# rdevooght/sequence-based-recommendations

Hardware: AMD Instinct MI355X
Metric: user-sequences/sec training (ML-1M shape, seq200 b256) at 1/2/4/8 GPUs (higher is better)
Workload: dtype f32; 1 GPU; c2: train.py -m RNN --r_t GRU --r_l 128 --max_length 200 -b 256 --loss CCE --u_m adam, N=3706 items, Zipf(1.0) ids, lengths=full, 256 rows per GPU; global_batch=256, seq_len=200, parallelism=dp1

## Files before the change

### sequence-based-recommendations_amd/csrc/sbr_api.hip

```cpp
#include "sbr_common.h"
#include <stdarg.h>
#include <stdio.h>
#include <string.h>
#include <algorithm>
#include <stdlib.h>
#include <math.h>
#include <array>
#include <atomic>
#include <chrono>

static thread_local std::string g_err;
void sbr_set_error(const char* fmt, ...) {
    char buf[1024];
    va_list ap; va_start(ap, fmt); vsnprintf(buf, sizeof(buf), fmt, ap); va_end(ap);
    g_err = buf;
}
extern "C" const char* sbr_last_error(void) { return g_err.c_str(); }
extern "C" int sbr_abi_version(void) { return SBR_ABI_VERSION; }


int sbr_build_layout(const sbr_config& cfg, Layout& lay, std::string& err) {
    char buf[256];
#define LFAIL(...) do { snprintf(buf, sizeof(buf), __VA_ARGS__); err = buf; return SBR_EINVAL; } while (0)
    if (cfg.abi_version != SBR_ABI_VERSION) LFAIL("abi_version %d != %d", cfg.abi_version, SBR_ABI_VERSION);
// ... 338 lines not shown
    h->sw = sbr_read_switches();
    const SbrSwitches& sw = h->sw;
    h->rpt = sw.rpt;
    if (h->rpt != 1 && h->rpt != 2 && h->rpt != 4 && h->rpt != 8 && h->rpt != 16) { h->rpt = 4; while (h->rpt < 16 && h->lay.Bp / h->rpt > 256) h->rpt <<= 1; }
    if (sw.tail_trace) {
        if (hipMalloc(&h->tail_trace, 16384 * sizeof(unsigned long long)) != hipSuccess) h->tail_trace = nullptr;
        else (void)hipMemset(h->tail_trace, 0, 16384 * sizeof(unsigned long long));
    }
    int prio_lo = 0, prio_hi = 0;
    (void)hipDeviceGetStreamPriorityRange(&prio_lo, &prio_hi);
    bool ok = true;
    for (hipStream_t* st : handle_streams(h)) ok = ok && hipStreamCreateWithPriority(st, hipStreamNonBlocking, prio_hi) == hipSuccess;
    for (hipEvent_t* ev : handle_events(h)) ok = ok && hipEventCreateWithFlags(ev, hipEventDisableTiming) == hipSuccess;
#if SBR_BB_STREAM
    ok = ok && hipStreamCreateWithPriority(&h->s_bb, hipStreamNonBlocking, SBR_BB_STREAM == 2 ? prio_lo : prio_hi) == hipSuccess;
#endif
    if (!ok || hipHostMalloc((void**)&h->lag_host, 8 * sizeof(float), hipHostMallocDefault) != hipSuccess) {
        sbr_set_error("side stream creation failed"); sbr_destroy(h); return SBR_EHIP;
    }
#if !SBR_BB_STREAM
    h->s_bb = h->side3;
#endif
    memset(h->lag_host, 0, 8 * sizeof(float));
    hipError_t e = hipMemsetAsync(h->arena, 0, h->lay.s_end * sizeof(float), h->stream);
    if (e == hipSuccess) e = hipStreamSynchronize(h->stream);
    if (e != hipSuccess) { sbr_set_error("arena initialisation failed: %s", hipGetErrorString(e)); sbr_destroy(h); return SBR_EHIP; }
    if (h->lay.n_at > 0) {
        std::vector<float> at(h->lay.n_at);
        const double lr = cfg->learning_rate, b1 = cfg->beta1, b2 = cfg->beta2;
        for (int t = 1; t <= h->lay.n_at; ++t) at[t - 1] = (float)(lr * sqrt(1.0 - pow(b2, (double)t)) / (1.0 - pow(b1, (double)t)));
        e = hipMemcpy(h->A(h->lay.a_at), at.data(), at.size() * sizeof(float), hipMemcpyHostToDevice);
        if (e != hipSuccess) { sbr_set_error("a_t table upload failed: %s", hipGetErrorString(e)); sbr_destroy(h); return SBR_EHIP; }
    }
    *out = h;
    return SBR_OK;
}

extern "C" void sbr_destroy(sbr_handle* h) {
    if (!h) return;
    (void)hipStreamSynchronize(h->stream);
    for (hipStream_t* st : handle_streams(h)) if (*st) (void)hipStreamSynchronize(*st);
    for (int r = 0; r < sbr_handle::kRing; ++r)
        for (int i = 0; i < SBR_N_PHASES; ++i) if (h->ev[r][i]) (void)hipEventDestroy(h->ev[r][i]);
    for (int r = 0; r < sbr_handle::kChain; ++r)
        for (int i = 0; i < 2; ++i) if (h->ev_ch[r][i]) (void)hipEventDestroy(h->ev_ch[r][i]);
    for (hipEvent_t* ev : handle_events(h)) if (*ev) (void)hipEventDestroy(*ev);
#if SBR_BB_STREAM
    if (h->s_bb) (void)hipStreamDestroy(h->s_bb);
#endif
    for (hipStream_t* st : handle_streams(h)) if (*st) (void)hipStreamDestroy(*st);
    if (h->lag_host) (void)hipHostFree(h->lag_host);
    if (h->own_arena && h->arena) (void)hipFree(h->arena);
    if (h->tail_trace) (void)hipFree(h->tail_trace);
    if (h->tail_slab_dev) (void)hipFree(h->tail_slab_dev);
    if (h->rank_scratch) (void)hipFree(h->rank_scratch);
    delete h;
}

extern "C" int sbr_num_params(const sbr_handle* h) { return h ? (int)h->descs.size() : SBR_EINVAL; }

extern "C" int sbr_param_shape(const sbr_handle* h, int i, int64_t dims[2], int* ndim) {
    CHECK_ARG(h && dims && ndim && i >= 0 && i < (int)h->descs.size(), "bad parameter index %d", i);
    const ParamDesc& d = h->descs[i];
    dims[0] = d.d0; dims[1] = d.ndim == 2 ? d.d1 : 1; *ndim = d.ndim;
    return SBR_OK;
}

static SbrSparseRows sparse_rows(sbr_handle* h, int b) {
    const SparseBlockLayout& sb = h->lay.sparse[b];
    SbrSparseRows r; memset(&r, 0, sizeof(r));
    r.npairs = sb.npairs; r.n_rows = sb.n_rows;
    for (int k = 0; k < sb.npairs; ++k) { r.off[k] = sb.off[k]; r.width[k] = sb.width[k]; r.stride[k] = sb.stride[k]; }
    r.p = h->P(0); r.g = h->Gd(0); r.s0 = h->St(0, 0); r.s1 = h->lay.n_state_arrays > 1 ? h->St(1, 0) : nullptr;
    r.last = (int*)h->A(sb.a_last);
    return r;
}
static SbrSparseUpd sparse_upd(sbr_handle* h) {
// ... 190 lines not shown
    const double geom = sbr_tail_geom(h->sw.tail_scatter_lds);
    SbrTChunks& tc = h->tail_bounds;
    tc.n = nc;
    tc.lo[0] = 0;
    double pw = h->sw.tail_scatter_lds ? (double)kTailFirst : 1.0;
    for (int c = 0; c < nc; ++c) {
        const int rem = y.T - tc.lo[c], left = nc - c;
        const int share = (rem + left - 1) / left;
        const int n_small = nc >= 4 ? nc / 2 : (nc - 1) / 2;
        int sz = (geom > 1.0 && c < n_small) ? std::min(share, std::max(1, (int)(pw + 0.5))) : (geom > 1.0 ? share : std::min(rem, ch));
        if (c == nc - 1) sz = rem;
        sz = std::max(1, std::min(sz, rem - (left - 1)));
        tc.lo[c + 1] = tc.lo[c] + sz;
        pw *= geom > 1.0 ? geom : 1.0;
    }
    for (int c = nc; c <= SBR_TCHUNKS_MAX; ++c) tc.lo[c] = y.T;
    return nc;
}

static int tail_next_epoch(sbr_handle* h) {
    h->prog_epoch = (h->prog_epoch + 1) & 0x7FFFF; if (!h->prog_epoch) h->prog_epoch = 1;
    return h->prog_epoch;
}
static int* tail_words(sbr_handle* h, int* nwaves) {
    *nwaves = (h->lay.Bp / rec_args(h, 0).rpt) * 8;
    return (int*)h->A(h->lay.a_prog);
}

static int tail_cost_scan(sbr_handle* h) {
    const Layout& y = h->lay;
    h->tail_cost_scanned = false;
    if (!h->sw.tail_scatter_lds) return SBR_OK;
    hipError_t e = hipSuccess;
    if (launch_scatter_cost_scan(h->side2, (const int*)h->A(y.a_soff), (int*)h->A(y.a_sP), y.cfg.input_size, h->tail_nc, y.T * y.Bp * y.F,
                                 y.G * y.layer[0].Hp, kTailScatterUnits, &e)) {
        if (e != hipSuccess) { sbr_set_error("HIP launch failed: %s", hipGetErrorString(e)); return SBR_EHIP; }
        h->tail_cost_scanned = true;
    }
    return SBR_OK;
}

static inline void chain_mark(sbr_handle* h, hipStream_t st, int dir, int which) {
    if (!h->chain_timing || h->ch_n >= sbr_handle::kChain) return;
    hipEvent_t& e = h->ev_ch[h->ch_n][which];
    if (!e && hipEventCreate(&e) != hipSuccess) { e = nullptr; return; }
    (void)hipEventRecord(e, st);
// ... 155 lines not shown
                SBR_LAUNCH(launch_sparse_catch_up_batch(s, sparse_rows(h, b), sparse_upd(h), h->bX, h->blen, y.T, y.Bp, y.F, (int)h->step_count));
    h->tail_nc = h->step_open ? tail_plan(h, &h->tail_ch) : 0;
    const bool training = h->step_open;
    h->step_open = false;
    h->tail_sorted = false;
    h->set_use[h->bb_set] = ++h->batch_seq; h->bb_unread = false;
    if (training) { if (h->train_fwd_open) h->bb_slow = 2; h->train_fwd_open = true; }
    h->cells_early = false;
    bool forked = false;
    if (training && h->sw.sparse_out_early && sparse_lazy(h) && y.S > 0 && y.cfg.loss != SBR_LOSS_CCE && !SBR_LOSS_IS_MARGIN(y.cfg.loss)) {
        int kb = -1;
        for (int b = 0; b < y.n_sparse; ++b) if (y.sparse[b].kind == 1) kb = b;
        if (kb >= 0) {
            SBR_HIP(hipEventRecord(h->ev_fork, s)); forked = true;
            SBR_HIP(hipStreamWaitEvent(h->side, h->ev_fork, 0));
            int* cells = (int*)h->A(y.a_cells);
            SBR_LAUNCH(launch_build_cells(h->side, h->btgt, h->bsmp, y.Bg, y.S, cells));
            SBR_LAUNCH(launch_sparse_catch_up_list(h->side, sparse_rows(h, kb), sparse_upd(h), cells, nullptr, y.C, y.C, (int)h->step_count));
            SBR_HIP(hipEventRecord(h->ev_cells, h->side));
            h->cells_early = true;
            h->side_pending = true;
        }
    }
    if (h->tail_nc >= 2 && h->sw.tail_overlap == 1) {
        if (!forked) SBR_HIP(hipEventRecord(h->ev_fork, s));
        SBR_HIP(hipStreamWaitEvent(h->side2, h->ev_fork, 0));
        SBR_LAUNCH(launch_scatter_sort(h->side2, h->bX, h->blen, y.T, y.Bp, y.F, y.cfg.input_size, (int*)h->A(y.a_scnt),
                                       (int*)h->A(y.a_soff), (int*)h->A(y.a_scur), (int*)h->A(y.a_sid), (int*)h->A(y.a_spos), 0,
                                       h->tail_ch, h->tail_nc, &h->tail_bounds, &h->scnt_zero_n));
        h->tail_sorted = true;
        { const int rc = tail_cost_scan(h); if (rc != SBR_OK) return rc; }
    }
    if (y.D == 2) return forward_bi(h);
    for (int l = 0; l < y.L; ++l) {
        const LayerLayout& ly = y.layer[l];
        const int GHp = y.G * ly.Hp;
        RecArgs ra = rec_args(h, l);
        if (l == 0 && y.E) {
            SBR_LAUNCH(launch_gather_concat(s, h->P(y.p_Emb), h->bX, h->A(y.a_emb), y.T, y.Bp, y.F, y.Ep));
            SBR_LAUNCH(launch_gemm(s, h->A(y.a_emb), ly.n_in_p, 1, h->P(ly.p_Win), GHp, 1, h->A(ly.a_xt), GHp, y.T * y.Bp, GHp,
                                   ly.n_in_p, h->P(ly.p_b), nullptr, 0, simple_gemm(h)));
            mark(h, 1);
        } else if (l == 0) {
            if (y.F == 1 && h->sw.fuse_gather && sbr_rec_fwd_can_fuse_gather(ra, simple_rec(h))) {
                ra.gX = h->bX; ra.gWin = h->P(ly.p_Win); ra.gbias = h->P(ly.p_b);
            } else {
                SBR_LAUNCH(launch_gather_xt(s, h->P(ly.p_Win), h->P(ly.p_b), h->bX, h->A(ly.a_xt), y.T, y.Bp,
                                            y.F, GHp, h->n_rows));
            }
            mark(h, 1);
        } else {
            const LayerLayout& lo = y.layer[l - 1];
            layer_gemm_hint(h, false, false);
            SBR_LAUNCH(launch_gemm(s, h->A(lo.a_hs) + (size_t)y.Bp * lo.Hp, lo.Hp, 1, h->P(ly.p_Win), GHp, 1, h->A(ly.a_xt), GHp,
                                   y.T * y.Bp, GHp, lo.Hp, h->P(ly.p_b), nullptr, 0, simple_gemm(h)));
        }
        if (l == 0 && h->tail_sorted) ra.fence_kb = kTailFenceKb;
        SBR_LAUNCH_CHAIN(0, s, launch_rec_forward(s, ra, simple_rec(h)));
    }
    mark(h, 2);
    h->fwd_done = true;
    return SBR_OK;
}

static float* h_last(sbr_handle* h) {
    const Layout& y = h->lay; const LayerLayout& ly = y.layer[(y.L - 1) * y.D];
    if (y.D == 2) return h->A(y.a_hcat);
    return h->A(ly.a_hs) + (size_t)y.T * y.Bp * ly.Hp;
}

static int side_join(sbr_handle* h) {
    if (h->tail_join_pending) {
        SBR_HIP(hipStreamWaitEvent(h->stream, h->ev_tail2, 0));
        SBR_HIP(hipStreamWaitEvent(h->stream, h->ev_tail, 0));
        h->tail_join_pending = false; h->side_pending = false;
    }
    if (h->side_pending) {
        SBR_HIP(hipEventRecord(h->ev_join, h->side));
        SBR_HIP(hipStreamWaitEvent(h->stream, h->ev_join, 0));
        h->side_pending = false;
    }
    return SBR_OK;
}

extern "C" int sbr_loss_backward_output(sbr_handle* h) {
    CHECK_ARG(h, "null handle");
    sbr_gemm_set_exact_f32((h->lay.cfg.flags & SBR_FLAG_F32_MFMA) != 0);
    if (!h->fwd_done) { sbr_set_error("sbr_loss_backward_output: call sbr_forward first"); return SBR_ESTATE; }
    const Layout& y = h->lay; hipStream_t s = h->stream, sd = h->side;
    const int R = h->n_rows, Hp = y.HLt, N = y.N;
    const bool sg = simple_gemm(h);
    h->grads_clean = false;
    h->dh_slabs_n = 0;
    float* hl = h_last(h);
    float* ws = h->A(y.a_ws);
    float* ws2 = h->A(y.a_ws2);
    const int* tgt = h->btgt;
    if (R < y.Bp) SBR_HIP(hipMemsetAsync(h->A(y.a_dhlast), 0, (size_t)y.Bp * Hp * sizeof(float), s));
    h->side_pending = true;
    h->fill_done = false;
    h->tail_gated = false; h->last_tail_gated = 0;
    bool fill_needed = false;
    if (!simple_rec(h))
        for (int l = 0; l < y.L * y.D; ++l) fill_needed = fill_needed || sbr_rec_cluster_ok(rec_args(h, l));
    auto side_batch_work = [&]() -> int {
        if (fill_needed) {
            for (int l = 0; l < y.L * y.D; ++l) {
                RecArgs a = rec_args(h, l);
                if (sbr_rec_cluster_ok(a)) SBR_LAUNCH(sbr_rec_bwd_cl_fill(sd, a));
            }
            SBR_HIP(hipEventRecord(h->ev_fill, sd)); h->fill_done = true;
        }
        if (h->tail_nc >= 2) {
            if (h->ev_lg_rec) SBR_HIP(hipStreamWaitEvent(h->side2, h->ev_lg_rec, 0));
            if (!h->tail_sorted) {
                SBR_LAUNCH(launch_scatter_sort(h->side2, h->bX, h->blen, y.T, y.Bp, y.F, y.cfg.input_size, (int*)h->A(y.a_scnt),
                                               (int*)h->A(y.a_soff), (int*)h->A(y.a_scur), (int*)h->A(y.a_sid), (int*)h->A(y.a_spos), 0,
                                               h->tail_ch, h->tail_nc, &h->tail_bounds, &h->scnt_zero_n));
                { const int rc = tail_cost_scan(h); if (rc != SBR_OK) return rc; }
            }
        } else if (!(y.cfg.flags & SBR_FLAG_ATOMIC_SCATTER) || y.E || y.n_sparse) {
            SBR_LAUNCH(launch_scatter_sort(sd, h->bX, h->blen, y.T, y.Bp, y.F,
                                           y.cfg.input_size, (int*)h->A(y.a_scnt), (int*)h->A(y.a_soff), (int*)h->A(y.a_scur),
                                           (int*)h->A(y.a_sid), (int*)h->A(y.a_spos), y.E ? 1 : 0, 0, 1, nullptr, &h->scnt_zero_n));
            if (y.D == 2 && !y.E)
                SBR_LAUNCH(launch_scatter_sort(sd, (const int*)h->A(y.a_Xr), h->blen, y.T, y.Bp, y.F, y.cfg.input_size,
                                               (int*)h->A(y.a_s2cnt), (int*)h->A(y.a_s2off), (int*)h->A(y.a_s2cur),
                                               (int*)h->A(y.a_s2sid), (int*)h->A(y.a_s2pos), 0));
            SBR_HIP(hipEventRecord(h->ev_sort, sd));
        }
        return SBR_OK;
    };
    if (fill_needed) {
        SBR_HIP(hipEventRecord(h->ev_fork, s));
        SBR_HIP(hipStreamWaitEvent(sd, h->ev_fork, 0));
        const int rc = side_batch_work(); if (rc != SBR_OK) return rc;
    }
    auto release_side = [&]() -> int {
        const bool mark3 = h->timing && ((h->timing_marks >> 3) & 1) && h->ev[h->ring_cur][3];
        if (kTailGateFirst && h->in_train_step && h->tail_nc >= 2 && h->sw.tail_overlap == 1 && h->tail_sorted && y.L == 1 && y.D == 1 && !fill_needed && !mark3) {
            int nwaves = 0;
            int* words = tail_words(h, &nwaves);
            SBR_LAUNCH(launch_tail_gate_wave(sd, words, nwaves, tail_next_epoch(h), y.T, (int*)h->A(y.a_fault)));
            h->tail_gated = true;
            h->ev_lg_rec = nullptr; h->ev_step_rec = h->ev_fork; h->lg_seq = h->batch_seq;
        } else {
            h->ev_lg_rec = h->ev_step_rec = record_shared(h, h->ev_lg, 3); h->lg_seq = h->batch_seq;
            SBR_HIP(hipStreamWaitEvent(sd, h->ev_lg_rec, 0));
        }
        return SBR_OK;
    };
    if (y.cfg.loss == SBR_LOSS_CCE || SBR_LOSS_IS_MARGIN(y.cfg.loss)) {
        float* lg = h->A(y.a_logits);
        const int Nl = (N + 3) & ~3;
        const bool bf16p = (y.cfg.flags & SBR_FLAG_BF16_PROJECTION) && !sg;
        int keep = 0;
        bool fold = false;
        if (!sg && y.D == 1 && R == y.Bp && !simple_rec(h)) {
            RecArgs ra = rec_args(h, y.L - 1);
            fold = sbr_rec_x6p_ok(ra) && !sbr_rec_cluster_ok(ra);
        }
        bool head_done = false;
        if (h->sw.head_fuse && y.cfg.loss == SBR_LOSS_CCE && !sg && !bf16p && !(y.cfg.flags & SBR_FLAG_F32_MFMA) && y.D == 1 && R == y.Bp) {
            int nsl = 0; hipError_t he = hipSuccess;
            h->head_epoch += 1; if (!h->head_epoch) h->head_epoch = 1;
            if (launch_head_cce(s, hl, h->P(y.p_WoutT), h->P(y.p_bout), tgt, h->bpop, lg, h->A(y.a_rowcost), ws, y.ws_floats,
                                (unsigned*)h->A(y.a_hstat), (int*)h->A(y.a_fault), y.Bp, N, Nl, Hp, y.Bg, h->head_epoch, h->sw.head_wait_ticks, &nsl, &he,
                                (y.cfg.flags & SBR_FLAG_PROFILE_REC) && (size_t)y.Bp * 16 >= 256 * 8 ? (unsigned long long*)h->A(y.a_prof) + (size_t)2 * (y.Bp / 16) * 16 * 8 : nullptr)) {
                SBR_LAUNCH(he);
                head_done = true;
// ... 186 lines not shown
            if (!gated) SBR_LAUNCH(launch_tail_gate(sd, words, nwaves, a.prog_epoch, y.T, a.fault));
            {
                hipError_t we = hipSuccess;
                if (!launch_gemm_slabs_x6_poll(sd, h->A(ly.a_hs), 1, ly.Hp, a.dxt, GHp, 1, ly.Hp, GHp, K, ws2, n_slabs, GHp, slab,
                                               gru ? a.dhi : nullptr, ly.Hp, gru ? 2 * ly.Hp : 0, &we, wg_f16 ? 2 : 3, 1.0f, wg_f16 ? 512.0f : 1.0f, pl)) {
                    sbr_set_error("overlapped tail: the weight-gradient GEMM rejected the shape"); return SBR_EINVAL;
                }
                SBR_LAUNCH(we);
            }
            if (gated) SBR_LAUNCH(launch_tail_gate_wave(s2, words, nwaves, a.prog_epoch, y.T, a.fault));
            else if (!serial) SBR_LAUNCH(launch_tail_gate(s2, words, nwaves, a.prog_epoch, y.T, a.fault));
            hipError_t se = hipSuccess;
            if (h->tail_cost_scanned && launch_scatter_lds_poll(s2, h->Gd(ly.p_Win), a.dxt, (const int*)h->A(y.a_sid), (const int*)h->A(y.a_spos),
                                                               (const int*)h->A(y.a_soff), (const int*)h->A(y.a_sP), y.cfg.input_size, tnc,
                                                               y.T * y.Bp * y.F, GHp, pl, h->tail_bounds, kTailScatterUnits, &se,
                                                               mon_in_units, a.t_lo)) {
                SBR_LAUNCH(se); h->last_scatter_form = 5;
            } else {
            h->last_scatter_form = 4;
            SBR_LAUNCH(launch_scatter_reduce_poll(s2, h->Gd(ly.p_Win), a.dxt, (const int*)h->A(y.a_sid), (const int*)h->A(y.a_spos),
                                                  (const int*)h->A(y.a_soff), y.cfg.input_size, tnc, CH, y.T * y.Bp * y.F, GHp, y.Bp, pl,
                                                  0, &h->tail_bounds, kTailShortChunks, !serial && kTailFenceKb > 0));
            }
            if (upd_here) SBR_LAUNCH(upd_on(s2, ly.p_Win, ly.p_b));
            SBR_HIP(hipEventRecord(h->ev_tail2, s2));
            if (upd_here && ly.p_peep - ly.p_Whid == slab && (slab & 3) == 0) {
                SBR_LAUNCH(launch_update_from_slabs(sd, y.cfg.updater, ws2, n_slabs, h->P(ly.p_Whid), h->St(0, ly.p_Whid),
                                                    s1a ? s1a + ly.p_Whid : nullptr, slab, y.cfg.learning_rate, y.cfg.rho, y.cfg.beta1,
                                                    y.cfg.beta2, (long)h->step_count + 1));
            } else {
                SBR_LAUNCH(launch_splitk_reduce(sd, ws2, n_slabs, ly.Hp, GHp, h->Gd(ly.p_Whid), GHp, nullptr));
                if (upd_here) SBR_LAUNCH(upd_on(sd, ly.p_Whid, ly.p_peep));
            }
            SBR_HIP(hipEventRecord(h->ev_tail, sd));
            SBR_LAUNCH(launch_rec_reduce_partials(s, a.part, nblk, y.G, ly.Hp, y.cfg.cell, h->Gd(ly.p_b), h->Gd(ly.p_peep),
                                                  h->Gd(ly.p_cinit), h->Gd(ly.p_hinit)));
            mark(h, 5);
            if (upd_here) {
                if (!out_early && h->og_recorded) SBR_HIP(hipStreamWaitEvent(s, h->ev_og, 0));
                SBR_LAUNCH(upd_on(s, ly.p_b, out_early ? y.p_split : y.n_params, ly.p_Whid - ly.p_b, ly.p_peep - ly.p_Whid));
                h->tail_updated = true;
            }
            if (h->deferred_join && !h->in_train_step && !serial) {
                h->tail_join_pending = true;
                mark(h, 6);
                continue;
            }
            SBR_HIP(hipStreamWaitEvent(s, h->ev_tail2, 0));
            mark(h, 6);
            SBR_HIP(hipStreamWaitEvent(s, h->ev_tail, 0));
            h->side_pending = false;
            continue;
        }
        hipEvent_t ev_chain_end = nullptr;
        if (nc > 1 || side_wgrad) {
            for (int c = 0; c < nc; ++c) {
                a.t_hi = (int)((long)y.T * (nc - c) / nc); a.t_lo = (int)((long)y.T * (nc - c - 1) / nc); a.chunk = c;
                SBR_LAUNCH_CHAIN(1, s, launch_rec_backward(s, a, false));
                ev_chain_end = record_shared(h, h->ev_chunk[c], (l == 0 && c == nc - 1) ? 4 : -1);
                SBR_HIP(hipStreamWaitEvent(sd, ev_chain_end, 0));
                const float* hsc = h->A(ly.a_hs) + (size_t)a.t_lo * y.Bp * ly.Hp;
                const int Kc = (a.t_hi - a.t_lo) * y.Bp;
                float* slabs = ws2 + (size_t)c * nsl * slab;
                const bool gru = y.cfg.cell == SBR_CELL_GRU;
                const float* dxc = a.dxt + (size_t)a.t_lo * y.Bp * GHp;
                const float* dhcc = gru ? a.dhi + (size_t)a.t_lo * y.Bp * ly.Hp : nullptr;
                hipError_t we = hipSuccess;
                if (sw == s && h->og_recorded) SBR_HIP(hipStreamWaitEvent(s, h->ev_og, 0));
// ... 752 lines not shown
        if (entries) *entries = off[y.cfg.input_size];
        if (rows) *rows = nr;
    }
    SBR_HIP(hipMemsetAsync(dW, 0, (size_t)y.cfg.input_size * GHp * sizeof(float), s));
    SBR_HIP(hipStreamSynchronize(s));
    h->tail_sorted = false;
    return SBR_OK;
}

extern "C" int sbr_query(sbr_handle* h, const char* what, int64_t* value) {
    CHECK_ARG(h && what && value, "null argument");
    const Layout& y = h->lay; const std::string w(what);
    if (w == "fused_gather") {
        RecArgs a = rec_args(h, 0);
        *value = (y.E == 0 && y.F == 1 && h->sw.fuse_gather && sbr_rec_fwd_can_fuse_gather(a, simple_rec(h))) ? 1 : 0;
    } else if (w == "rows_per_workgroup") *value = h->rpt;
    else if (w == "head_fused") {
        int cc = 0, cw = 0; size_t lds = 0;
        *value = (h->sw.head_fuse && y.cfg.loss == SBR_LOSS_CCE && !simple_gemm(h) && !(y.cfg.flags & (SBR_FLAG_BF16_PROJECTION | SBR_FLAG_F32_MFMA)) &&
                  y.D == 1 && y.B == y.Bp && sbr_head_plan(y.Bp, y.N, y.HLt, &cc, &cw, &lds) && (size_t)cc * y.Bp * y.HLt <= y.ws_floats) ? cc : 0;
    }
    else if (w == "head_sampled") *value = head_sampled_taken(h, y.B) ? 1 : 0;
    else if (w == "scatter_form") *value = h->last_scatter_form;
    else if (w == "tail_gate_first") *value = h->last_tail_gated;
    else if (w == "rank_select") *value = h->last_rank_select;
    else if (w == "rank_sort") *value = h->last_rank_sort;
    else if (w == "cluster_rank_form") *value = h->last_cluster_rank_form;
    else if (w == "row_aware_update") *value = h->last_row_aware ? 1 : 0;
    else if (w == "cluster") { RecArgs a = rec_args(h, (y.L - 1) * y.D); *value = (!simple_rec(h) && sbr_rec_cluster_ok(a)) ? 1 : 0; }
    else if (w == "rec_kernel") {
        RecArgs a = rec_args(h, (y.L - 1) * y.D);
        *value = simple_rec(h) ? 0 : sbr_rec_cluster_ok(a) ? 1 : sbr_rec_x6p_ok(a) ? 2 : sbr_rec_x6q_ok(a) ? 3 : 4;
    }
    else if (w.rfind("rec_products_", 0) == 0 || w.rfind("rec_rows_", 0) == 0 || w.rfind("rec_workgroups_", 0) == 0) {
        const bool bwd = w.size() > 4 && w.compare(w.size() - 4, 4, "_bwd") == 0;
        RecArgs a = rec_args(h, (y.L - 1) * y.D);
        const bool cl = !simple_rec(h) && sbr_rec_cluster_ok(a), xp = sbr_rec_x6p_ok(a), xq = sbr_rec_x6q_ok(a);
        const bool x6 = cl || xp || xq || (!a.f32_mfma && (a.Hp == 32 || a.Hp == 64 || a.Hp == 128));
        int products = 0, rows = 16, wgs = y.Bp / 16;
        if (!simple_rec(h) && x6) {
            const bool f16 = (xp || cl || xq) && (bwd ? sbr_rec_f16_bwd(a) : sbr_rec_f16_fwd(a));
            products = f16 ? (xp && !cl ? sbr_rec_x6p_f16_terms() : 3) : 6;
            if (cl && sbr_rec_c16_ok(a)) { rows = 16; wgs = (y.Bp / 16) * (a.Hp / 16); }
            else if (cl) { rows = bwd ? sbr_rec_cluster_bwd_rows(a) : SBR_CL_ROWS; wgs = (y.Bp / rows) * (a.Hp == 256 ? 8 : 32); }
            else { rows = a.rpt; wgs = y.Bp / a.rpt; }
        }
// ... 69 lines not shown
```

### sequence-based-recommendations_amd/csrc/sbr_batch.hip

```cpp
#include "sbr_common.h"
#include <algorithm>
#include <unordered_map>

struct sbr_dataset {
    int64_t n_users, nnz; int n_items;
    hipStream_t stream;
    int* d_items; long long* d_off;
    float* d_popdb; double* d_cdf;
    int* d_rate;
    int shuffle_targets;
    int *d_items_n, *d_rate_n, *d_len_n; int noised; int64_t max_len;
    std::vector<int> len_n32;
    std::vector<int64_t> len_cur;
    int host_rows, hr_targets; uint64_t hr_seed, hr_pass;
    std::vector<float> keep_prob;
    std::vector<int> h_items, h_items_cur;
    std::vector<int64_t> h_off;
    std::vector<int> hr_user, hr_split, hr_tgt, hr_pu, hr_ps, hr_pt;
    int *d_hr_user, *d_hr_split, *d_hr_tgt; size_t cap_hru, cap_hrs, cap_hrt;
    std::vector<int64_t> len;
    std::vector<int> pend_user, pend_k;
    std::vector<int> seg_user, seg_k, seg_row0, seg_batch, batch_begin;
    int *d_seg_user, *d_seg_k, *d_seg_row0, *d_batch_begin; size_t cap_su, cap_sk, cap_sr, cap_bb;
    int *d_split, *d_rowuser; size_t cap_rows;
// ... 563 lines not shown
    if (seg_user) *seg_user = d->seg_user.data();
    if (seg_k) *seg_k = d->seg_k.data();
    if (seg_row0) *seg_row0 = d->seg_row0.data();
    if (seg_batch) *seg_batch = d->seg_batch.data();
    return SBR_OK;
}

extern "C" int sbr_build_batch(sbr_handle* h, sbr_dataset* d, int64_t batch, uint64_t seed) {
    CHECK_ARG(h && d, "null handle / dataset");
    const Layout& y = h->lay;
    CHECK_ARG(y.F == 1 || (y.F == 2 && d->d_rate && y.cfg.input_size == y.N + 10),
              "the native batch builder covers the item index and, with ratings attached (sbr_dataset_set_options), the rating index");
    CHECK_ARG(d->n_items == y.N && (y.cfg.input_size == y.N || y.F == 2), "dataset has %d items, the model %d", d->n_items, y.N);
    CHECK_ARG(!d->shuffle_targets || y.NT <= 16 || d->host_rows, "shuffled targets: at most 16 targets per row on the device");
    CHECK_ARG(d->batch_size == y.Bg, "the pass was planned for batches of %d rows, the model's global batch is %d", d->batch_size, y.Bg);
    CHECK_ARG(batch >= 0 && batch < d->n_batches, "batch %lld outside the planned pass [0,%lld)", (long long)batch, (long long)d->n_batches);
    CHECK_ARG(d->stream == h->stream, "dataset and engine must share one stream");
    hipStream_t s = h->s_bb;
    const int set = h->bb_set ^ 1;
    if (h->train_fwd_open) h->bb_slow = 2;
    if (h->bb_unread && h->bb_slow == 0) h->bb_slow = 1;
    if (h->bb_slow == 0 && h->ev_step_rec && h->lg_seq > h->set_use[set]) {
        SBR_HIP(hipStreamWaitEvent(s, h->ev_step_rec, 0));
    } else {
        hipStream_t all[4] = {h->stream, h->side, h->side2, h->side3};
        for (hipStream_t q : all) { SBR_HIP(hipEventRecord(h->ev_bbw, q)); SBR_HIP(hipStreamWaitEvent(s, h->ev_bbw, 0)); }
        if (h->bb_slow > 0) --h->bb_slow;
    }
    if ((size_t)y.Bg > d->cap_rows) {
        (void)hipFree(d->d_split); (void)hipFree(d->d_rowuser); d->d_split = d->d_rowuser = nullptr;
        SBR_HIP(hipMalloc(&d->d_split, (size_t)y.Bg * sizeof(int)));
        SBR_HIP(hipMalloc(&d->d_rowuser, (size_t)y.Bg * sizeof(int)));
        d->cap_rows = y.Bg;
    }
    const unsigned long long sd = seed ^ (0x9E3779B97F4A7C15ull * (unsigned long long)(batch + 1));
    const int* len_n = d->noised ? d->d_len_n : nullptr;
    const int* src_items = d->noised ? d->d_items_n : d->d_items;
    const int* src_rate = d->noised && d->d_rate ? d->d_rate_n : d->d_rate;
    const int *split = d->d_split, *rowuser = d->d_rowuser, *tgtpos = nullptr;
    if (d->host_rows) {
        CHECK_ARG(d->hr_targets == y.NT, "the rows were planned for %d targets, the model has %d", d->hr_targets, y.NT);
        split = d->d_hr_split + batch * y.Bg; rowuser = d->d_hr_user + batch * y.Bg; tgtpos = d->d_hr_tgt + batch * (int64_t)y.Bg * y.NT;
    } else {
        const int sb = d->batch_begin[batch], se = d->batch_begin[batch + 1];
        bb_split_kernel<<<se - sb, 256, 0, s>>>(d->d_off, len_n, d->d_seg_user, d->d_seg_k, d->d_seg_row0, sb, sd, d->d_split, d->d_rowuser);
        SBR_LAUNCH(hipGetLastError());
// ... 19 lines not shown
```

### sequence-based-recommendations_amd/csrc/sbr_common.h

```cpp
#pragma once
#include <hip/hip_runtime.h>
#include <stdint.h>
#include <stddef.h>
#include <string>
#include <vector>
#include "../../include/sbr_rnn.h"

#define SBR_BWD_CHUNKS 4
#define SBR_ALIGN_FLOATS 64

static inline size_t sbr_align(size_t n_floats) { return (n_floats + SBR_ALIGN_FLOATS - 1) / SBR_ALIGN_FLOATS * SBR_ALIGN_FLOATS; }
static inline int sbr_gates(int cell) { return cell == SBR_CELL_LSTM ? 4 : (cell == SBR_CELL_GRU ? 3 : 1); }
static inline int sbr_pad_hidden(int H) {
    if (H <= 16) return 16;
    if (H <= 32) return 32;
    if (H <= 64) return 64;
    if (H <= 128) return 128;
    if (H <= 256) return 256;
    if (H <= 512) return 512;
    return (H + 63) / 64 * 64;
}

struct LayerLayout {
    int H, Hp, G;
// ... 85 lines not shown
struct ParamDesc { std::string name; int layer; int kind; int gate; int64_t d0, d1; int ndim; };
void sbr_param_descs(const Layout& lay, std::vector<ParamDesc>& out);

#define SBR_TCHUNKS_MAX 9
struct SbrTChunks { int n; int lo[SBR_TCHUNKS_MAX + 1]; };
static inline SbrTChunks sbr_uniform_tchunks(int tch, int n) {
    SbrTChunks tc; tc.n = tch > 0 ? n : 0;
    for (int c = 0; c <= SBR_TCHUNKS_MAX; ++c) tc.lo[c] = tch * (c < n ? c : n);
    return tc;
}
constexpr int kWgradSlices = 256;
constexpr int kWgradX6Wgs = 512;
constexpr int kTailChunksMax = 8;
constexpr int kTailPubEvery = 2;
constexpr int kTailShortChunks = 3;
constexpr int kTailFenceKb = 124;
constexpr int kTailFirst = 6;
constexpr int kTailScatterUnits = 192;
constexpr int kTailGemmGroups = 64;
constexpr int kTailSlabMax = 512;
constexpr double kTailSlabGrowth = 0.35;
constexpr bool kTailGateFirst = true;
constexpr int kTailGateSleep = 32;
static inline double sbr_tail_geom(int scatter_lds) { return scatter_lds ? 1.6 : 2.6; }
constexpr int kRankThreads = 1024;
constexpr int kRankLdsRow = 32768;
constexpr int kRankSortLds = 2048;

#define HEAD_WAIT_TICKS 6000ull
struct SbrSwitches {
    int rpt = 0;
    int bwd_chunks = 1;
    int cluster = 1;
    int cl_linear = 0;
    int cl16 = 1;
    int c16_two_level = 1;
    int x6_pipe = 1;
    int x6_f16 = 1;
    int x6_f16_bwd = 1;
    int fuse_gather = 1;
    int gemm_f16 = 1;
    int wgrad_f16 = 1;
    int tail_overlap = 1;
    int tail_scatter_lds = 1;
    int tail_trace = 0;
    int scat_range = 1;
// ... 47 lines not shown
    uint64_t lg_seq = 0;
    bool bb_unread = false;
    bool train_fwd_open = false;
    int bb_slow = 0;
    int n_rows = 0;
    int64_t step_count = 0;
    bool have_batch = false, fwd_done = false;
    bool grads_clean = false;
    bool timing = false;
    unsigned timing_marks = 0;
    int tail_nc = 0, tail_ch = 0;
    SbrTChunks tail_bounds = {};
    unsigned long long* tail_trace = nullptr;
    bool tail_sorted = false;
    void* rank_scratch = nullptr; size_t rank_scratch_bytes = 0; int last_rank_select = 0, last_rank_sort = 0;
    int last_cluster_rank_form = 0;
    int last_tail_gated = -1;
    int last_scatter_form = -1; bool last_row_aware = false;
    bool tail_cost_scanned = false;
    int scnt_zero_n = 0;
    std::vector<int> tail_slab_host; int* tail_slab_dev = nullptr; int tail_slab_key[2] = {0, 0};
    int prog_epoch = 0;
    bool tail_gated = false;
    hipEvent_t ev_step_rec = nullptr;
    bool tail_updated = false;
    bool tail_join_pending = false;
    bool step_open = false;
    hipEvent_t ev_lg_rec = nullptr;
    bool tail_swapped = false;
    unsigned marks_shared = 0;
    static const int kRing = 64;
    hipEvent_t ev[kRing][SBR_N_PHASES] = {};
    int ring_used = 0;
    int ring_cur = 0;
    static const int kChain = 256;
    hipEvent_t ev_ch[kChain][2] = {};
    unsigned char ch_dir[kChain] = {};
    int ch_n = 0;
    bool chain_timing = false;
    float* P(size_t off) const { return arena + lay.s_params + off; }
    float* Gd(size_t off) const { return arena + lay.s_grads + off; }
    float* St(int k, size_t off) const { return arena + lay.s_state + (size_t)k * lay.n_params + off; }
    float* A(size_t off) const { return arena + lay.s_act + off; }
    float* cost_ptr() const { return arena + lay.s_grads + lay.n_params; }
};

// ... 22 lines not shown
    sbr_set_error("%s failed: %s (%s:%d)", #call, hipGetErrorString(e_), __FILE__, __LINE__); return SBR_EHIP; } } while (0)

#define CHECK_ARG(cond, ...) do { if (!(cond)) { sbr_set_error(__VA_ARGS__); return SBR_EINVAL; } } while (0)
#define SBR_LAUNCH(call) do { hipError_t e_ = (call); if (e_ != hipSuccess) { \
    sbr_set_error("%s failed: %s (%s:%d)", #call, hipGetErrorString(e_), __FILE__, __LINE__); return SBR_EHIP; } } while (0)

#define SBR_DYN_LDS(KERNEL, LDS) do { static int sbr_dyn_lds_set_ = -1; if ((int)(LDS) > sbr_dyn_lds_set_) { \
        (void)hipFuncSetAttribute((const void*)KERNEL, hipFuncAttributeMaxDynamicSharedMemorySize, (int)(LDS)); sbr_dyn_lds_set_ = (int)(LDS); } } while (0)
#define SBR_DONE_COPIES 32
#define SBR_DONE_STRIDE 1088
struct SbrPoll { const int* words; int n; int* done; int epoch; int rows_per_step; int* fault; int n_small, k_small;
                 unsigned long long* trace; const int* slab_lo; int n_slabs; };

hipError_t launch_gather_xt(hipStream_t s, const float* Win, const float* bias, const int* X, float* xt,
                            int T, int Bp, int F, int GHp, int n_rows_in);
hipError_t launch_scatter_rows(hipStream_t s, float* dWin, const float* dxt, const int* X, const int* len,
                               int T, int Bp, int F, int GHp);
hipError_t launch_scatter_sort(hipStream_t s, const int* X, const int* len, int T, int Bp, int F, int n_ids, int* cnt,
                               int* offs, int* cur, int* sid, int* spos, int concat = 0, int tch = 0, int n_tchunks = 1, const SbrTChunks* bounds = nullptr,
                               int* cnt_zero_n = nullptr);
int sbr_scatter_lds_ids();
hipError_t launch_tail_gate(hipStream_t s, const int* progress, int n, int epoch, int target, int* fault);
hipError_t launch_tail_gate_wave(hipStream_t s, const int* progress, int n, int epoch, int target, int* fault);
hipError_t launch_gather_concat(hipStream_t s, const float* Wemb, const int* X, float* out, int T, int Bp, int F, int Ep);
hipError_t launch_rev_rows_int(hipStream_t s, const int* X, const int* len, int* Xr, int T, int Bp, int F);
hipError_t launch_rev_rows(hipStream_t s, const float* src, const int* len, float* dst, int T, int Bp, int W);
hipError_t launch_cat_outputs(hipStream_t s, const float* hs_f, const float* hs_b, const int* len, float* cat, int T, int Bp, int Hp);
hipError_t launch_hcat(hipStream_t s, const float* hf, const float* hb, float* out, int Bp, int Hp);
hipError_t launch_split_cols(hipStream_t s, const float* src, float* a, float* b, int rows, int Hp);
hipError_t launch_uncat(hipStream_t s, const float* f, const float* r, const int* len, float* out_f, float* out_b, int T, int Bp,
                        int W, int Hp);
bool launch_scatter_range(hipStream_t s, float* dWin, const float* dxt, const int* sid, const int* spos, const int* offs, int n_ids,
                          int GHp, float* part, int* part_id, int n_ranges, hipError_t* err);
#define SBR_SCAT_RANGES 512
bool launch_scatter_wide(hipStream_t s, float* dWin, const float* dxt, const int* sid, const int* spos, const int* offs, int n_ids,
                         int max_entries, int GHp, float* part, int* aux, int n_slots, hipError_t* err);
struct SbrScatStep { float* p; float* s0; float* s1; int* last; int updater, t_to; float lr, rho, b1, b2, a_t; };
static inline int sbr_scatter_wide_slots(size_t max_entries) { return (int)(max_entries / 64 + max_entries / 65 + 2); }
hipError_t launch_scatter_reduce(hipStream_t s, float* dWin, const float* dxt, const int* sid, const int* spos,
                                 const int* offs, int n_ids, int max_entries, int GHp, int Bp, int key_lo = 0, bool accumulate = false, int acc_chunk = 32);
bool launch_scatter_cost_scan(hipStream_t s, const int* offs, int* P, int n_ids, int n_tchunks, int max_entries, int GHp, int units,
                              hipError_t* err);
hipError_t launch_tail_monitor(hipStream_t s, const SbrPoll& poll, int t_lo);
bool launch_scatter_lds_poll(hipStream_t s, float* dWin, const float* dxt, const int* sid, const int* spos, const int* offs, const int* P,
                             int n_ids, int n_tchunks, int max_entries, int GHp, const SbrPoll& poll, const SbrTChunks& bounds,
                             int units, hipError_t* err, bool monitor = false, int t_lo = 0);
// ... 24 lines not shown
    float* state;
    float* part;
    int rpt;
    int xt_blocked;
    int x6_pipe;
    int x6_f16, x6_f16_bwd;
    int cl16, c16_two_level;
    const int* gX;
    const float* gWin;
    int n_in;
    const float* gbias;
    int f32_mfma;
    unsigned long long* prof;
    int cluster;
    int cl_linear;
    int* fault;
    int sentinel_done;
    int* clx;
    void* xh;
    float* pring;
    int epoch;
    int relu;
    int* progress; int prog_every; int prog_epoch;
    int fence_kb;
};
static inline bool sbr_rec_f16_fwd(const RecArgs& a) { return a.x6_f16 && !a.relu; }
static inline bool sbr_rec_f16_bwd(const RecArgs& a) { return a.x6_f16_bwd && a.clip > 0.0f && a.clip <= 100.0f; }
#define SBR_CL_ROWS 8
#define SBR_C16_RING 2
#define SBR_X6P_FUSE_MAX_T 4096
bool sbr_rec_cluster_ok(const RecArgs& a);
int sbr_rec_cluster_bwd_rows(const RecArgs& a);
hipError_t launch_rec_forward_cl(hipStream_t s, const RecArgs& a);
hipError_t launch_rec_backward_cl(hipStream_t s, const RecArgs& a);
bool sbr_rec_x6p_ok(const RecArgs& a);
bool sbr_rec_x6p_fuse_ok(const RecArgs& a);
int sbr_rec_x6p_f16_terms();
bool sbr_rec_x6p_tail_ok(const RecArgs& a);
hipError_t launch_rec_forward_x6p(hipStream_t s, const RecArgs& a);
hipError_t launch_rec_backward_x6p(hipStream_t s, const RecArgs& a);
bool sbr_rec_x6q_ok(const RecArgs& a);
hipError_t launch_rec_forward_x6q(hipStream_t s, const RecArgs& a);
hipError_t launch_rec_backward_x6q(hipStream_t s, const RecArgs& a);
hipError_t sbr_rec_bwd_cl_fill(hipStream_t s, const RecArgs& a);
bool sbr_rec_c16_ok(const RecArgs& a);
size_t sbr_rec_c16_ring_floats(int Bp, int Hp);
// ... 114 lines not shown
```

### sequence-based-recommendations_amd/csrc/sbr_misc.hip

```cpp
#include "sbr_common.h"
#include "sbr_rec_p.h"
#include <math.h>

typedef float f32x4 __attribute__((ext_vector_type(4)));

__device__ __forceinline__ float wave_sum(float v) {
#pragma unroll
    for (int o = 32; o > 0; o >>= 1) v += __shfl_xor(v, o);
    return v;
}
__device__ __forceinline__ float wave_max(float v) {
#pragma unroll
    for (int o = 32; o > 0; o >>= 1) v = fmaxf(v, __shfl_xor(v, o));
    return v;
}
__device__ __forceinline__ float block_sum(float v, float* red) {
    v = wave_sum(v);
    __syncthreads();
    if ((threadIdx.x & 63) == 0) red[threadIdx.x >> 6] = v;
    __syncthreads();
    float s = 0.0f;
    for (int w = 0; w < (int)(blockDim.x >> 6); ++w) s += red[w];
    return s;
}
// ... 1161 lines not shown
}

__global__ void __launch_bounds__(64) tail_gate_wave_kernel(const int* __restrict__ progress, int n, int epoch, int target, int* __restrict__ fault) {
    const unsigned long long t0 = wall_clock64();
    auto passed = [&](int v) { return (v >> 12) == epoch && (v & 0xfff) <= target; };
    for (;;) {
        if (passed(__hip_atomic_load(progress, __ATOMIC_RELAXED, __HIP_MEMORY_SCOPE_AGENT))) break;
        if (wall_clock64() - t0 > SBR_POLL_TICKS) { if (threadIdx.x == 0) atomicOr(fault, 8); return; }
        __builtin_amdgcn_s_sleep(kTailGateSleep);
    }
    for (;;) {
        bool ok = true;
#pragma unroll 8
        for (int i = 0; i < n; i += 64)
            ok = passed(__hip_atomic_load(progress + min(i + (int)threadIdx.x, n - 1), __ATOMIC_RELAXED, __HIP_MEMORY_SCOPE_AGENT)) && ok;
        if (__all(ok)) break;
        if (wall_clock64() - t0 > SBR_POLL_TICKS) { if (threadIdx.x == 0) atomicOr(fault, 8); return; }
        __builtin_amdgcn_s_sleep(8);
    }
}
hipError_t launch_tail_gate_wave(hipStream_t s, const int* progress, int n, int epoch, int target, int* fault) {
    if (n < 1) return hipErrorInvalidValue;
    tail_gate_wave_kernel<<<1, 64, 0, s>>>(progress, n, epoch, target, fault);
    return hipGetLastError();
}

__global__ void scatter_rows_kernel(float* __restrict__ dWin, const f32x4* __restrict__ dxt, const int* __restrict__ X,
                                    const int* __restrict__ len, int T, int Bp, int F, int R4) {
    const size_t total = (size_t)T * Bp * R4;
    for (size_t i = (size_t)blockIdx.x * blockDim.x + threadIdx.x; i < total; i += (size_t)gridDim.x * blockDim.x) {
        const int f4 = (int)(i % R4);
        const size_t pos = i / R4;
        const int b = (int)(pos % Bp), t = (int)(pos / Bp);
        if (t >= len[b]) continue;
        const f32x4 v = dxt[i];
        const int* ids = X + ((size_t)b * T + t) * F;
        for (int f = 0; f < F; ++f) {
            float* dst = dWin + ((size_t)ids[f] * R4 + f4) * 4;
            atomicAdd(dst + 0, v[0]); atomicAdd(dst + 1, v[1]); atomicAdd(dst + 2, v[2]); atomicAdd(dst + 3, v[3]);
        }
    }
}

hipError_t launch_scatter_rows(hipStream_t s, float* dWin, const float* dxt, const int* X, const int* len, int T,
                               int Bp, int F, int GHp) {
    const int R4 = GHp / 4;
// ... 588 lines not shown
```

### sequence-based-recommendations_amd/csrc/sbr_rec_p.hip

```cpp
#include "sbr_rec_p.h"

#ifndef X6P_BWD_NS
#define X6P_BWD_NS 4
#endif
#ifndef X6P_BWD_LA
#define X6P_BWD_LA 3
#endif
#ifndef X6P_FWD_V2
#define X6P_FWD_V2 6
#endif
#ifndef X6P_BWD_DEFER
#define X6P_BWD_DEFER 0
#endif
#ifndef X6P_FWD_TOK
#define X6P_FWD_TOK 1
#endif
#ifndef X6P_G4
#define X6P_G4 1
#endif
#ifndef X6P_SPEC1
#define X6P_SPEC1 0
#endif
#ifndef X6P_H1_AT
#define X6P_H1_AT 0
// ... 40 lines not shown
}

}

template <int CELL, bool FUSE, bool PROF, bool F16>
__global__ void __launch_bounds__(512) rec_fwd_x6p(RecArgs a) {
    using OPV = std::conditional_t<F16, f16x8, bf16x8>;
    constexpr int NP = F16 ? 2 : 3;
    constexpr bool PK = F16 && X6P_PACK;
    constexpr bool SP = PK && X6P_SPARSE;
    constexpr int G = Gates<CELL>::G, KB = KBH, GHP = G * HP;
    static_assert(G <= 3 || F16, "three W_hid planes of four gates do not fit the register file: an LSTM runs on the two fp16 planes only");
    constexpr int HROW = HP * 2 + 32, PLANEB = R * HROW, BUFB = 3 * PLANEB;
    extern __shared__ __attribute__((aligned(16))) char smem_p[];
    char* hbuf = smem_p;
    int* cnt = (int*)(hbuf + 2 * BUFB);
    int* tok = cnt + 4;
    const int lane = threadIdx.x & 63, wave = __builtin_amdgcn_readfirstlane(threadIdx.x >> 6);
    const int j = lane & 15, q = lane >> 4;
    const int row = blockIdx.x * R + q;
    const int u = wave * 16 + j;
    const int T = a.T, Bp = a.Bp;
    if (threadIdx.x < 8) cnt[threadIdx.x] = 0;
    const bool roleA = wave < 4;
    int spin_limit = X6P_SPIN_LIMIT;
    const unsigned lds_tok = (unsigned)(size_t)(tok + (wave & 3));
    const int one = 1;

    const int mylen = a.len[row];
    int tmax = mylen;
    tmax = max(tmax, __shfl_xor(tmax, 16));
    tmax = __builtin_amdgcn_readfirstlane(max(tmax, __shfl_xor(tmax, 32)));

    OPV W1[SP ? 1 : G][SP ? 1 : KB], W2[SP ? 1 : G][SP ? 1 : KB], W3[F16 ? 1 : G][F16 ? 1 : KB];
    f16x16 WS[SP ? G : 1][SP ? KB : 1];
    if constexpr (SP) {
#pragma unroll
        for (int g = 0; g < G; ++g)
#pragma unroll
            for (int kb = 0; kb < KB; ++kb)
#pragma unroll
                for (int r = 0; r < 8; ++r) {
                    const float sc = (CELL == CELL_GRU && g < 2) ? X6P_NLOG2E : 1.0f;
                    float w = sc * a.Whid[(size_t)(kb * 32 + 16 * (r >> 2) + 4 * q + (r & 3)) * GHP + g * HP + u];
                    _Float16 b1, b2;
                    asm("" : "+v"(w));
// ... 920 lines not shown
```

Baseline: 818,300 user-sequences/s.

## Replace stream events with device-side step words for fork and join gating

Adds device-memory step words written by tiny kernels (or by the forward recurrent kernel at start) and polled by a one-wave gate kernel. These replace hipEvent fork/join dependencies between the main and side streams around the early scatter sort and the tail weight updates. The early sort now launches after the forward recurrence, gated on the recurrence having started, and the batch-buffer wait polls the word. The aim is to cut event-based cross-stream synchronisation latency. In exchange it adds spin-wait kernels that occupy a CU slot, relies on relaxed atomics for ordering, and risks timeout faults if kernels are not co-resident.

```diff
diff --git a/sequence-based-recommendations_amd/csrc/sbr_api.hip b/sequence-based-recommendations_amd/csrc/sbr_api.hip
--- a/sequence-based-recommendations_amd/csrc/sbr_api.hip
+++ b/sequence-based-recommendations_amd/csrc/sbr_api.hip
@@ -384,6 +384,9 @@
     h->s_bb = h->side3;
 #endif
     memset(h->lag_host, 0, 8 * sizeof(float));
+    if (hipMalloc(&h->step_words, 160 * sizeof(int)) != hipSuccess || hipMemset(h->step_words, 0, 160 * sizeof(int)) != hipSuccess) {
+        sbr_set_error("step boundary words: allocation failed"); sbr_destroy(h); return SBR_EHIP;
+    }
     hipError_t e = hipMemsetAsync(h->arena, 0, h->lay.s_end * sizeof(float), h->stream);
     if (e == hipSuccess) e = hipStreamSynchronize(h->stream);
     if (e != hipSuccess) { sbr_set_error("arena initialisation failed: %s", hipGetErrorString(e)); sbr_destroy(h); return SBR_EHIP; }
@@ -415,6 +418,7 @@
     if (h->own_arena && h->arena) (void)hipFree(h->arena);
     if (h->tail_trace) (void)hipFree(h->tail_trace);
     if (h->tail_slab_dev) (void)hipFree(h->tail_slab_dev);
+    if (h->step_words) (void)hipFree(h->step_words);
     if (h->rank_scratch) (void)hipFree(h->rank_scratch);
     delete h;
 }
@@ -651,6 +655,8 @@
     h->prog_epoch = (h->prog_epoch + 1) & 0x7FFFF; if (!h->prog_epoch) h->prog_epoch = 1;
     return h->prog_epoch;
 }
+static int step_next_epoch(int* e) { *e = (*e + 1) & 0x7FFFFFFF; if (!*e) *e = 1; return *e; }
+static bool step_boundary_marks(const sbr_handle* h) { return h->timing && (h->timing_marks & ((1u << 0) | (1u << 6))); }
 static int* tail_words(sbr_handle* h, int* nwaves) {
     *nwaves = (h->lay.Bp / rec_args(h, 0).rpt) * 8;
     return (int*)h->A(h->lay.a_prog);
@@ -852,15 +858,26 @@
             h->side_pending = true;
         }
     }
-    if (h->tail_nc >= 2 && h->sw.tail_overlap == 1) {
-        if (!forked) SBR_HIP(hipEventRecord(h->ev_fork, s));
-        SBR_HIP(hipStreamWaitEvent(h->side2, h->ev_fork, 0));
+    auto early_sort = [&]() -> int {
         SBR_LAUNCH(launch_scatter_sort(h->side2, h->bX, h->blen, y.T, y.Bp, y.F, y.cfg.input_size, (int*)h->A(y.a_scnt),
                                        (int*)h->A(y.a_soff), (int*)h->A(y.a_scur), (int*)h->A(y.a_sid), (int*)h->A(y.a_spos), 0,
                                        h->tail_ch, h->tail_nc, &h->tail_bounds, &h->scnt_zero_n));
         h->tail_sorted = true;
-        { const int rc = tail_cost_scan(h); if (rc != SBR_OK) return rc; }
-    }
+        return tail_cost_scan(h);
+    };
+    h->fork_gated = false; h->step_word_epoch = 0;
+    const bool sort_early = h->tail_nc >= 2 && h->sw.tail_overlap == 1;
+    bool fork_gate = false;
+    if (kStepForkGate && sort_early && h->in_train_step && y.L == 1 && y.D == 1 && !forked && !step_boundary_marks(h) && !simple_rec(h)) {
+        const RecArgs r0 = rec_args(h, 0);
+        fork_gate = sbr_rec_x6p_ok(r0) && !sbr_rec_cluster_ok(r0);
+    }
+    if (sort_early && !fork_gate) {
+        if (!forked) SBR_HIP(hipEventRecord(h->ev_fork, s));
+        SBR_HIP(hipStreamWaitEvent(h->side2, h->ev_fork, 0));
+        { const int rc = early_sort(); if (rc != SBR_OK) return rc; }
+    }
+    if (training) h->last_fork_gate = fork_gate;
     if (y.D == 2) return forward_bi(h);
     for (int l = 0; l < y.L; ++l) {
         const LayerLayout& ly = y.layer[l];
@@ -885,8 +902,14 @@
             SBR_LAUNCH(launch_gemm(s, h->A(lo.a_hs) + (size_t)y.Bp * lo.Hp, lo.Hp, 1, h->P(ly.p_Win), GHp, 1, h->A(ly.a_xt), GHp,
                                    y.T * y.Bp, GHp, lo.Hp, h->P(ly.p_b), nullptr, 0, simple_gemm(h)));
         }
-        if (l == 0 && h->tail_sorted) ra.fence_kb = kTailFenceKb;
+        if (l == 0 && (h->tail_sorted || fork_gate)) ra.fence_kb = kTailFenceKb;
+        if (fork_gate) { ra.start_word = h->step_words + 128; ra.start_epoch = step_next_epoch(&h->fork_epoch); }
         SBR_LAUNCH_CHAIN(0, s, launch_rec_forward(s, ra, simple_rec(h)));
+        if (fork_gate) {
+            h->fork_gated = true; h->step_word_epoch = h->fork_epoch;
+            SBR_LAUNCH(launch_step_gate(h->side2, h->step_words + 128, nullptr, h->fork_epoch, (int*)h->A(y.a_fault)));
+            { const int rc = early_sort(); if (rc != SBR_OK) return rc; }
+        }
     }
     mark(h, 2);
     h->fwd_done = true;
@@ -930,6 +953,7 @@
     h->side_pending = true;
     h->fill_done = false;
     h->tail_gated = false; h->last_tail_gated = 0;
+    h->last_join_gate = 0;
     bool fill_needed = false;
     if (!simple_rec(h))
         for (int l = 0; l < y.L * y.D; ++l) fill_needed = fill_needed || sbr_rec_cluster_ok(rec_args(h, l));
@@ -973,9 +997,10 @@
             int* words = tail_words(h, &nwaves);
             SBR_LAUNCH(launch_tail_gate_wave(sd, words, nwaves, tail_next_epoch(h), y.T, (int*)h->A(y.a_fault)));
             h->tail_gated = true;
-            h->ev_lg_rec = nullptr; h->ev_step_rec = h->ev_fork; h->lg_seq = h->batch_seq;
+            h->ev_lg_rec = nullptr; h->ev_step_rec = h->fork_gated ? nullptr : h->ev_fork; h->lg_seq = h->batch_seq;
         } else {
             h->ev_lg_rec = h->ev_step_rec = record_shared(h, h->ev_lg, 3); h->lg_seq = h->batch_seq;
+            h->step_word_epoch = 0;
             SBR_HIP(hipStreamWaitEvent(sd, h->ev_lg_rec, 0));
         }
         return SBR_OK;
@@ -1208,7 +1233,11 @@
                                                   (const int*)h->A(y.a_soff), y.cfg.input_size, tnc, CH, y.T * y.Bp * y.F, GHp, y.Bp, pl,
                                                   0, &h->tail_bounds, kTailShortChunks, !serial && kTailFenceKb > 0));
             }
+            const bool join_gate = kStepJoinGate && upd_here && !serial && !step_boundary_marks(h);
+            if (join_gate) step_next_epoch(&h->join_epoch);
+            h->last_join_gate = join_gate;
             if (upd_here) SBR_LAUNCH(upd_on(s2, ly.p_Win, ly.p_b));
+            if (join_gate) SBR_LAUNCH(launch_step_word(s2, h->step_words + 96, h->join_epoch));
             SBR_HIP(hipEventRecord(h->ev_tail2, s2));
             if (upd_here && ly.p_peep - ly.p_Whid == slab && (slab & 3) == 0) {
                 SBR_LAUNCH(launch_update_from_slabs(sd, y.cfg.updater, ws2, n_slabs, h->P(ly.p_Whid), h->St(0, ly.p_Whid),
@@ -1218,6 +1247,7 @@
                 SBR_LAUNCH(launch_splitk_reduce(sd, ws2, n_slabs, ly.Hp, GHp, h->Gd(ly.p_Whid), GHp, nullptr));
                 if (upd_here) SBR_LAUNCH(upd_on(sd, ly.p_Whid, ly.p_peep));
             }
+            if (join_gate) SBR_LAUNCH(launch_step_word(sd, h->step_words + 32, h->join_epoch));
             SBR_HIP(hipEventRecord(h->ev_tail, sd));
             SBR_LAUNCH(launch_rec_reduce_partials(s, a.part, nblk, y.G, ly.Hp, y.cfg.cell, h->Gd(ly.p_b), h->Gd(ly.p_peep),
                                                   h->Gd(ly.p_cinit), h->Gd(ly.p_hinit)));
@@ -1230,6 +1260,11 @@
             if (h->deferred_join && !h->in_train_step && !serial) {
                 h->tail_join_pending = true;
                 mark(h, 6);
+                continue;
+            }
+            if (join_gate) {
+                SBR_LAUNCH(launch_step_gate(s, h->step_words + 32, h->step_words + 96, h->join_epoch, a.fault));
+                h->side_pending = false;
                 continue;
             }
             SBR_HIP(hipStreamWaitEvent(s, h->ev_tail2, 0));
@@ -2028,6 +2063,8 @@
     }
     else if (w == "head_sampled") *value = head_sampled_taken(h, y.B) ? 1 : 0;
     else if (w == "scatter_form") *value = h->last_scatter_form;
+    else if (w == "step_join_gate") *value = h->last_join_gate;
+    else if (w == "step_fork_gate") *value = h->last_fork_gate;
     else if (w == "tail_gate_first") *value = h->last_tail_gated;
     else if (w == "rank_select") *value = h->last_rank_select;
     else if (w == "rank_sort") *value = h->last_rank_sort;
diff --git a/sequence-based-recommendations_amd/csrc/sbr_batch.hip b/sequence-based-recommendations_amd/csrc/sbr_batch.hip
--- a/sequence-based-recommendations_amd/csrc/sbr_batch.hip
+++ b/sequence-based-recommendations_amd/csrc/sbr_batch.hip
@@ -609,6 +609,8 @@
     if (h->bb_unread && h->bb_slow == 0) h->bb_slow = 1;
     if (h->bb_slow == 0 && h->ev_step_rec && h->lg_seq > h->set_use[set]) {
         SBR_HIP(hipStreamWaitEvent(s, h->ev_step_rec, 0));
+    } else if (h->bb_slow == 0 && h->step_word_epoch && h->step_words && h->lg_seq > h->set_use[set]) {
+        SBR_LAUNCH(launch_step_gate(s, h->step_words + 128, nullptr, h->step_word_epoch, (int*)h->A(y.a_fault)));
     } else {
         hipStream_t all[4] = {h->stream, h->side, h->side2, h->side3};
         for (hipStream_t q : all) { SBR_HIP(hipEventRecord(h->ev_bbw, q)); SBR_HIP(hipStreamWaitEvent(s, h->ev_bbw, 0)); }
diff --git a/sequence-based-recommendations_amd/csrc/sbr_common.h b/sequence-based-recommendations_amd/csrc/sbr_common.h
--- a/sequence-based-recommendations_amd/csrc/sbr_common.h
+++ b/sequence-based-recommendations_amd/csrc/sbr_common.h
@@ -131,6 +131,8 @@
 constexpr double kTailSlabGrowth = 0.35;
 constexpr bool kTailGateFirst = true;
 constexpr int kTailGateSleep = 32;
+constexpr bool kStepJoinGate = true;
+constexpr bool kStepForkGate = true;
 static inline double sbr_tail_geom(int scatter_lds) { return scatter_lds ? 1.6 : 2.6; }
 constexpr int kRankThreads = 1024;
 constexpr int kRankLdsRow = 32768;
@@ -224,6 +226,11 @@
     std::vector<int> tail_slab_host; int* tail_slab_dev = nullptr; int tail_slab_key[2] = {0, 0};
     int prog_epoch = 0;
     bool tail_gated = false;
+    int* step_words = nullptr;
+    int join_epoch = 0, fork_epoch = 0;
+    bool fork_gated = false;
+    int last_join_gate = -1, last_fork_gate = -1;
+    int step_word_epoch = 0;
     hipEvent_t ev_step_rec = nullptr;
     bool tail_updated = false;
     bool tail_join_pending = false;
@@ -292,6 +299,8 @@
 int sbr_scatter_lds_ids();
 hipError_t launch_tail_gate(hipStream_t s, const int* progress, int n, int epoch, int target, int* fault);
 hipError_t launch_tail_gate_wave(hipStream_t s, const int* progress, int n, int epoch, int target, int* fault);
+hipError_t launch_step_gate(hipStream_t s, const int* w0, const int* w1, int epoch, int* fault);
+hipError_t launch_step_word(hipStream_t s, int* word, int epoch);
 hipError_t launch_gather_concat(hipStream_t s, const float* Wemb, const int* X, float* out, int T, int Bp, int F, int Ep);
 hipError_t launch_rev_rows_int(hipStream_t s, const int* X, const int* len, int* Xr, int T, int Bp, int F);
 hipError_t launch_rev_rows(hipStream_t s, const float* src, const int* len, float* dst, int T, int Bp, int W);
@@ -362,6 +371,7 @@
     int epoch;
     int relu;
     int* progress; int prog_every; int prog_epoch;
+    int* start_word; int start_epoch;
     int fence_kb;
 };
 static inline bool sbr_rec_f16_fwd(const RecArgs& a) { return a.x6_f16 && !a.relu; }
diff --git a/sequence-based-recommendations_amd/csrc/sbr_misc.hip b/sequence-based-recommendations_amd/csrc/sbr_misc.hip
--- a/sequence-based-recommendations_amd/csrc/sbr_misc.hip
+++ b/sequence-based-recommendations_amd/csrc/sbr_misc.hip
@@ -1207,6 +1207,30 @@
 hipError_t launch_tail_gate_wave(hipStream_t s, const int* progress, int n, int epoch, int target, int* fault) {
     if (n < 1) return hipErrorInvalidValue;
     tail_gate_wave_kernel<<<1, 64, 0, s>>>(progress, n, epoch, target, fault);
+    return hipGetLastError();
+}
+
+__global__ void __launch_bounds__(64) step_gate_kernel(const int* __restrict__ w0, const int* __restrict__ w1, int epoch, int* __restrict__ fault) {
+    const unsigned long long t0 = wall_clock64();
+    for (;;) {
+        const int a = __hip_atomic_load(w0, __ATOMIC_RELAXED, __HIP_MEMORY_SCOPE_AGENT);
+        const int b = w1 ? __hip_atomic_load(w1, __ATOMIC_RELAXED, __HIP_MEMORY_SCOPE_AGENT) : epoch;
+        if (a == epoch && b == epoch) break;
+        if (wall_clock64() - t0 > SBR_POLL_TICKS) { if (threadIdx.x == 0) atomicOr(fault, 8); return; }
+        __builtin_amdgcn_s_sleep(8);
+    }
+}
+hipError_t launch_step_gate(hipStream_t s, const int* w0, const int* w1, int epoch, int* fault) {
+    if (!w0 || !epoch) return hipErrorInvalidValue;
+    step_gate_kernel<<<1, 64, 0, s>>>(w0, w1, epoch, fault);
+    return hipGetLastError();
+}
+__global__ void __launch_bounds__(64) step_word_kernel(int* __restrict__ word, int epoch) {
+    if (threadIdx.x == 0) __hip_atomic_store(word, epoch, __ATOMIC_RELAXED, __HIP_MEMORY_SCOPE_AGENT);
+}
+hipError_t launch_step_word(hipStream_t s, int* word, int epoch) {
+    if (!word || !epoch) return hipErrorInvalidValue;
+    step_word_kernel<<<1, 64, 0, s>>>(word, epoch);
     return hipGetLastError();
 }
 
diff --git a/sequence-based-recommendations_amd/csrc/sbr_rec_p.hip b/sequence-based-recommendations_amd/csrc/sbr_rec_p.hip
--- a/sequence-based-recommendations_amd/csrc/sbr_rec_p.hip
+++ b/sequence-based-recommendations_amd/csrc/sbr_rec_p.hip
@@ -86,6 +86,8 @@
     const int u = wave * 16 + j;
     const int T = a.T, Bp = a.Bp;
     if (threadIdx.x < 8) cnt[threadIdx.x] = 0;
+    if (a.start_word && blockIdx.x == 0 && threadIdx.x == 0)
+        __hip_atomic_store(a.start_word, a.start_epoch, __ATOMIC_RELAXED, __HIP_MEMORY_SCOPE_AGENT);
     const bool roleA = wave < 4;
     int spin_limit = X6P_SPIN_LIMIT;
     const unsigned lds_tok = (unsigned)(size_t)(tok + (wave & 3));
```

Measured after the change: 864,300 user-sequences/s (median of 6 runs). +5.6%, better.
